# NIRVANALAN/CVPR23-E3DGE

Measured on AMD Instinct MI355X. Metric: rendered_rays_per_sec_64x64x24, higher is better.
Workload: dtype f32 (operands split f16 hi+lo, 3 f16 MFMA products, fp32 accumulate)

## Files before the change

cvpr23-e3dge_amd/csrc/siren16.h:

```cpp
#pragma once
#include "siren_common.h"

namespace e3dge {

typedef float f32x4v __attribute__((ext_vector_type(4)));

constexpr int k16Threads = 512;
constexpr int k16Tiles = 16;
constexpr int k16Steps = 8;
constexpr int k16ChunkFloats = 16 * kWidth;
constexpr int k16Chunks = kBigLayers * k16Tiles;
constexpr int k16NBuf = 4;
constexpr int k16Slots = 2;
constexpr int k16Ring = 2;

constexpr int k16LdsW = 0;
constexpr int k16LdsFilm = k16LdsW + k16NBuf * k16ChunkFloats;
constexpr int k16LdsHead = k16LdsFilm + 9 * 2 * kWidth;
constexpr int k16LdsW0 = k16LdsHead + kHeadFloats;
constexpr int k16LdsVrec = k16LdsW0 + 3 * kWidth;
constexpr int k16LdsFeat = k16LdsVrec + 2 * 4 * kWidth;
constexpr int k16LdsPart = k16LdsFeat + kRMax * kFPitch;
constexpr int k16LdsAlpha = ((k16LdsPart + 8 * k16Slots * kWidth + 3) / 4) * 4;
constexpr int k16LdsWgt = k16LdsAlpha + kTilePts;
constexpr int k16LdsZ = k16LdsWgt + kTilePts;
constexpr int k16LdsPts = k16LdsZ + kTilePts;
constexpr int k16LdsRgb = k16LdsPts + kTilePts * 3;
constexpr int k16LdsState = k16LdsRgb + kTilePts * 3;
constexpr int k16LdsWq = ((k16LdsState + kRMax * kStateStride + 3) / 4) * 4;
constexpr int k16LdsVd = k16LdsWq + 8 * k16Slots * 16;
constexpr int k16LdsFloats = k16LdsVd + 8 * 16 * 4;
constexpr int k16LdsBytes = k16LdsFloats * 4;
static_assert(k16LdsBytes <= 160 * 1024, "LDS budget");
static_assert((k16LdsFilm % 4) == 0 && (k16LdsHead % 4) == 0 && (k16LdsW0 % 4) == 0 && (k16LdsVrec % 4) == 0, "alignment");

__device__ __forceinline__ void save_st4(float* p, const f32x4v& v) {
    __builtin_nontemporal_store(v, reinterpret_cast<f32x4v*>(p));
}
__device__ __forceinline__ f32x4v mfma16x16(u32x4 a, u32x4 b, f32x4v c) {
    return __builtin_amdgcn_mfma_f32_16x16x32_f16(__builtin_bit_cast(half8, a), __builtin_bit_cast(half8, b), c, 0, 0, 0);
}
__device__ __forceinline__ f32x4v zero4() { return f32x4v{0.f, 0.f, 0.f, 0.f}; }
template <int HI> __device__ __forceinline__ float fma_mix_h(unsigned p, float w, float acc) {
    float r;
    if (HI) asm("v_fma_mix_f32 %0, %1, %2, %3 op_sel:[1,0,0] op_sel_hi:[1,0,0]" : "=v"(r) : "v"(p), "v"(w), "v"(acc));
    else asm("v_fma_mix_f32 %0, %1, %2, %3 op_sel:[0,0,0] op_sel_hi:[1,0,0]" : "=v"(r) : "v"(p), "v"(w), "v"(acc));
    return r;
}
__device__ __forceinline__ float act16_get(const u32x4 (&aH)[k16Steps], const u32x4 (&aL)[k16Steps], int t, int r) {
    const int g = t >> 1, w = 2 * (t & 1) + (r >> 1);
    return (r & 1) ? f16hi(aH[g][w]) + f16hi(aL[g][w]) : f16lo(aH[g][w]) + f16lo(aL[g][w]);
}
template <int CTRL> __device__ __forceinline__ float dpp16(float x) {
    return __builtin_bit_cast(float, __builtin_amdgcn_update_dpp(0, __builtin_bit_cast(int, x), CTRL, 0xf, 0xf, true));
}
__device__ __forceinline__ float row_sum16(float x) {
    x += dpp16<0x128>(x);
    x += dpp16<0x124>(x);
    x += dpp16<0x122>(x);
    x += dpp16<0x121>(x);
    return x;
}

__device__ __forceinline__ float sum_over_q(float x) {
    const unsigned u = __builtin_bit_cast(unsigned, x);
    const auto r = __builtin_amdgcn_permlane16_swap(u, u, false, false);
    const float y = __builtin_bit_cast(float, (unsigned)r[0]) + __builtin_bit_cast(float, (unsigned)r[1]);
    const unsigned v = __builtin_bit_cast(unsigned, y);
    const auto t = __builtin_amdgcn_permlane32_swap(v, v, false, false);
    return __builtin_bit_cast(float, (unsigned)t[0]) + __builtin_bit_cast(float, (unsigned)t[1]);
}

template <int CTRL, int ROW_MASK> __device__ __forceinline__ float dpp_or(float ident, float x) {
    return __builtin_bit_cast(float, __builtin_amdgcn_update_dpp(__builtin_bit_cast(int, ident), __builtin_bit_cast(int, x), CTRL, ROW_MASK, 0xf, false));
}
__device__ __forceinline__ float wave_incl_prod(float x) {
    x = __fmul_rn(x, dpp_or<0x111, 0xf>(1.0f, x));
    x = __fmul_rn(x, dpp_or<0x112, 0xf>(1.0f, x));
    x = __fmul_rn(x, dpp_or<0x114, 0xf>(1.0f, x));
    x = __fmul_rn(x, dpp_or<0x118, 0xf>(1.0f, x));
    x = __fmul_rn(x, dpp_or<0x142, 0xa>(1.0f, x));
    x = __fmul_rn(x, dpp_or<0x143, 0xc>(1.0f, x));
    return x;
}
__device__ __forceinline__ float wave_sum_last(float x) {
    x = __fadd_rn(x, dpp_or<0x111, 0xf>(0.0f, x));
    x = __fadd_rn(x, dpp_or<0x112, 0xf>(0.0f, x));
    x = __fadd_rn(x, dpp_or<0x114, 0xf>(0.0f, x));
    x = __fadd_rn(x, dpp_or<0x118, 0xf>(0.0f, x));
    x = __fadd_rn(x, dpp_or<0x142, 0xa>(0.0f, x));
    x = __fadd_rn(x, dpp_or<0x143, 0xc>(0.0f, x));
    return __builtin_bit_cast(float, __builtin_amdgcn_readlane(__builtin_bit_cast(int, x), 63));
}

struct ChunkPipe16 {
    const char* img;
    uint32_t voff, lds_base;
    int idx, buf, use_buf, count;
    float* wbuf;
    const float* wcur;
    const float* wnxt;
    __device__ __forceinline__ void init(float* wbuf_, const float* image, int wave, int lane, int count_ = k16Chunks) {
        const int wave_u = __builtin_amdgcn_readfirstlane(wave);
        wbuf = wbuf_;
        count = count_;
        img = reinterpret_cast<const char*>(image) + wave_u * 2048;
        voff = (uint32_t)lane * 16u;
        lds_base = (uint32_t)(size_t)(__attribute__((address_space(3))) float*)wbuf_ + (uint32_t)wave_u * 2048u;
        idx = 0; buf = 0; use_buf = 0;
        wcur = wbuf_; wnxt = wbuf_ + k16ChunkFloats;
    }
    __device__ __forceinline__ void issue_chunk() {
        const char* s = img + (size_t)idx * (k16ChunkFloats * 4);
        const uint32_t d = lds_base + (uint32_t)buf * (k16ChunkFloats * 4);
        glds16_saddr<0>(s, voff, d);
        glds16_saddr<1024>(s, voff, d);
        idx = (idx + 1 == count) ? 0 : idx + 1;
        buf = (buf + 1 == k16NBuf) ? 0 : buf + 1;
    }
    __device__ __forceinline__ void prime() {
        issue_chunk(); issue_chunk(); issue_chunk();
    }
#ifdef E3DGE_PHASE_TIMING
    unsigned long long t_vm = 0, t_bar = 0;
#endif
    template <bool STRICT> __device__ __forceinline__ void sync() {
#ifdef E3DGE_PHASE_TIMING
        const unsigned long long c0 = __builtin_readcyclecounter();
#endif
        if (STRICT) asm volatile("s_waitcnt vmcnt(0)" ::: "memory");
        else asm volatile("s_waitcnt vmcnt(2)" ::: "memory");
#ifdef E3DGE_PHASE_TIMING
        const unsigned long long c1 = __builtin_readcyclecounter();
#endif
        __syncthreads();
#ifdef E3DGE_PHASE_TIMING
        t_vm += c1 - c0; t_bar += __builtin_readcyclecounter() - c1;
#endif
    }
    __device__ __forceinline__ void advance() {
        use_buf = (use_buf + 1 == k16NBuf) ? 0 : use_buf + 1;
        wcur = wnxt;
        wnxt = wbuf + ((use_buf + 1 == k16NBuf) ? 0 : use_buf + 1) * k16ChunkFloats;
    }
};

#ifdef E3DGE_16_TRACE
__device__ unsigned long long g_trace16[2][24];
#define TRACE16_STAMP(i) do { if (trace) asm volatile("s_memtime %0" : "=s"(tstamp[i])); } while (0)
#else
#define TRACE16_STAMP(i) do { } while (0)
#endif

template <bool TRANSPOSED, int RING = k16Ring, class Epi, class Hook>
__device__ __forceinline__ void tile16(ChunkPipe16& pipe, int lane, const u32x4 (&aH)[k16Steps], const u32x4 (&aL)[k16Steps],
                                       f32x4v& acc, f32x4v& accb, u32x4 (&ringH)[RING], u32x4 (&ringL)[RING], Epi&& epi,
                                       Hook&& hook, int sbuf = -1, [[maybe_unused]] int trace = 0) {
#ifdef E3DGE_16_TRACE
    unsigned long long tstamp[24];
#endif
    const u32x4* __restrict__ wp = reinterpret_cast<const u32x4*>(sbuf >= 0 ? pipe.wbuf + sbuf * k16ChunkFloats : pipe.wcur) + lane;
    const u32x4* __restrict__ wn = reinterpret_cast<const u32x4*>(sbuf >= 0 ? pipe.wbuf + ((sbuf + 1) % k16NBuf) * k16ChunkFloats : pipe.wnxt) + lane;
#pragma unroll
    for (int g = 0; g < k16Steps; ++g) {
        const int ga = g + RING - 1;
        TRACE16_STAMP(3 * g);
        ringH[ga % RING] = (ga < k16Steps) ? wp[(ga * 2 + 0) * 64] : wn[((ga - k16Steps) * 2 + 0) * 64];
        ringL[ga % RING] = (ga < k16Steps) ? wp[(ga * 2 + 1) * 64] : wn[((ga - k16Steps) * 2 + 1) * 64];
        __builtin_amdgcn_sched_barrier(0);
        const u32x4 wh = ringH[g % RING], wl = ringL[g % RING];
        f32x4v& x0 = (g & 1) ? accb : acc;
        f32x4v& x1 = (g & 1) ? acc : accb;
        if (!TRANSPOSED) {
            x0 = mfma16x16(wh, aH[g], x0);
            x1 = mfma16x16(wl, aH[g], x1);
            x0 = mfma16x16(wh, aL[g], x0);
        } else {
            x0 = mfma16x16(aH[g], wh, x0);
            x1 = mfma16x16(aH[g], wl, x1);
            x0 = mfma16x16(aL[g], wh, x0);
        }
        TRACE16_STAMP(3 * g + 1);
        if (g == 1) hook();
        epi(g);
        TRACE16_STAMP(3 * g + 2);
    }
#ifdef E3DGE_16_TRACE
    if (trace) {
        asm volatile("s_waitcnt lgkmcnt(0)" ::: "memory");
        if ((threadIdx.x & 63) == 0)
            for (int i = 0; i < 24; ++i) g_trace16[trace - 1][i] = tstamp[i];
    }
#endif
}

#ifndef E3DGE_16_HELPERS_ONLY
#ifdef E3DGE_PHASE_TIMING
#define PHASE16(i) do { if (MODE == 0 && blockIdx.x == 0 && tid == 0 && sub < 3) tstamp[sub * 6 + (i)] = __builtin_readcyclecounter(); } while (0)
#else
#define PHASE16(i) do { } while (0)
#endif

constexpr int64_t k16SlabWords = 8 * 2 * 64;

template <int MODE, bool SAVE, int CACHE = 0>
__global__ void __launch_bounds__(k16Threads) siren16_kernel(const SirenK a) {
    static_assert(CACHE == 0 || (MODE == 0 && !SAVE), "the backbone hand-over exists for inference renders only");
    extern __shared__ __attribute__((aligned(16))) float smem[];
    float* const wbuf = smem + k16LdsW;
    float* const film_s = smem + k16LdsFilm;
    float* const head_s = smem + k16LdsHead;
    float* const w0_s = smem + k16LdsW0;
    float* const vrec_s = smem + k16LdsVrec;
    float* const feat_acc = smem + k16LdsFeat;
    float* const part = smem + k16LdsPart;
    float* const alpha_s = smem + k16LdsAlpha;
    float* const wgt_s = smem + k16LdsWgt;
    float* const z_s = smem + k16LdsZ;
    float* const pts_s = smem + k16LdsPts;
    float* const rgb_s = smem + k16LdsRgb;
    float* const state = smem + k16LdsState;

    const int tid_k = threadIdx.x;
#ifdef E3DGE_PHASE_TIMING
    const unsigned long long t_entry = __builtin_readcyclecounter();
    unsigned long long t_loop0 = 0, t_loop1 = 0;
#endif
    int b, npts, n_sub;
    int pix0 = 0, nrays = 0;
    long long pt0 = 0;
    const int S = (MODE == 0) ? a.S : 1;
    if (MODE == 0) {
        b = blockIdx.x / a.tiles_per_img;
        const int tile = blockIdx.x - b * a.tiles_per_img;
        const int HW = a.H * a.Wd;
        pix0 = tile * a.R;
        nrays = min(a.R, HW - pix0);
        npts = nrays * S;
    } else {
        b = blockIdx.x / a.wgs_per_img;
        const int wg = blockIdx.x - b * a.wgs_per_img;
        pt0 = (long long)wg * a.subtiles_per_wg * kTilePts;
        const long long rem = a.n_pts - pt0;
        npts = (int)(rem < (long long)a.subtiles_per_wg * kTilePts ? rem : (long long)a.subtiles_per_wg * kTilePts);
    }
    n_sub = (npts + kTilePts - 1) / kTilePts;

    const float* __restrict__ packed = a.packed;
    const float* __restrict__ film_g = a.film + (int64_t)b * 9 * 2 * kWidth;
    ChunkPipe16 pipe;
    if (CACHE == 2) pipe.init(wbuf, packed + kOffBig16b + (int64_t)(kBigLayers - 1) * k16Tiles * k16ChunkFloats, tid_k >> 6, tid_k & 63, k16Tiles);
    else pipe.init(wbuf, packed + kOffBig16b, tid_k >> 6, tid_k & 63);
    pipe.prime();
    constexpr int kFilmIt = (9 * kWidth + k16Threads - 1) / k16Threads;
    constexpr int kHeadIt = (kHeadFloats + k16Threads - 1) / k16Threads;
    constexpr int kColIt = (3 * kWidth + k16Threads - 1) / k16Threads;
    float ld_gm[kFilmIt], ld_bt[kFilmIt], ld_bias[kFilmIt], ld_head[kHeadIt], ld_w0[kColIt], ld_vt[kColIt];
#pragma unroll
    for (int j = 0; j < kFilmIt; ++j) {
        const int i = tid_k + j * k16Threads, l = i >> 8, n = i & 255;
        ld_gm[j] = ld_bt[j] = ld_bias[j] = 0.0f;
        if (i < 9 * kWidth) {
            ld_gm[j] = film_g[(l * 2 + 0) * kWidth + n];
            ld_bt[j] = film_g[(l * 2 + 1) * kWidth + n];
            ld_bias[j] = packed[kOffBias + l * kWidth + n];
        }
    }
#pragma unroll
    for (int j = 0; j < kHeadIt; ++j) {
        const int i = tid_k + j * k16Threads;
        ld_head[j] = (i < kHeadFloats) ? packed[kOffWSigma + i] : 0.0f;
    }
#pragma unroll
    for (int j = 0; j < kColIt; ++j) {
        const int i = tid_k + j * k16Threads, c = i >> 8, n = i & 255;
        const int src = ((n >> 5) * 2 + (c >> 1)) * 64 + (c & 1) * 32 + (n & 31);
        ld_w0[j] = ld_vt[j] = 0.0f;
        if (i < 3 * kWidth) { ld_w0[j] = packed[kOffFirst + src]; ld_vt[j] = packed[kOffVTail + src]; }
    }
#pragma unroll
    for (int j = 0; j < kFilmIt; ++j) {
        const int i = tid_k + j * k16Threads, l = i >> 8, n = i & 255;
        if (i < 9 * kWidth) {
            const float gm = ld_gm[j], bt = ld_bt[j];
            const float g_s = (l >= 1) ? gm * (1.0f / kW16Scale) : gm;
            const float b_s = __fadd_rn(__fmul_rn(gm, ld_bias[j]), bt);
            film_s[(l * 2 + 0) * kWidth + n] = g_s;
            film_s[(l * 2 + 1) * kWidth + n] = b_s;
            if (l == 8) { vrec_s[4 * n + 0] = g_s; vrec_s[4 * n + 1] = b_s; }
        }
    }
#pragma unroll
    for (int j = 0; j < kHeadIt; ++j) {
        const int i = tid_k + j * k16Threads;
        if (i < kHeadFloats) {
            head_s[i] = ld_head[j];
            const int c = (i >> 8) - 1, n = i & 255;
            if (c >= 0 && c < 3) vrec_s[(c == 2 ? 4 * kWidth : 0) + 4 * n + (c == 2 ? 0 : 2 + c)] = ld_head[j];
        }
    }
#pragma unroll
    for (int j = 0; j < kColIt; ++j) {
        const int i = tid_k + j * k16Threads, c = i >> 8, n = i & 255;
        if (i < 3 * kWidth) {
            w0_s[i] = ld_w0[j];
            vrec_s[4 * kWidth + 4 * n + 1 + c] = ld_vt[j] * kW16Scale;
        }
    }
    float cw[12] = {0}, focal = 1.f, nearv = 0.f, farv = 0.f;
    if (MODE == 0) {
#pragma unroll
        for (int i = 0; i < 12; ++i) cw[i] = a.c2w[b * 12 + i];
        focal = a.focal[b]; nearv = a.near[b]; farv = a.far[b];
        for (int i = tid_k; i < kRMax * kStateStride; i += k16Threads) state[i] = 0.0f;
        for (int i = tid_k; i < kRMax * kFPitch; i += k16Threads) feat_acc[i] = 0.0f;
    }
    const float* __restrict__ film = film_s;

    asm volatile("s_waitcnt vmcnt(0)" ::: "memory");
    __syncthreads();
    u32x4 ringH[k16Ring], ringL[k16Ring];
    {
        const int lane0 = tid_k & 63;
#pragma unroll
        for (int g = 0; g < k16Ring - 1; ++g) {
            ringH[g] = reinterpret_cast<const u32x4*>(pipe.wcur)[(g * 2 + 0) * 64 + lane0];
            ringL[g] = reinterpret_cast<const u32x4*>(pipe.wcur)[(g * 2 + 1) * 64 + lane0];
        }
    }

#ifdef E3DGE_16_TRACE
    auto trace_sel = [&](int L, int t) {
        const int w = __builtin_amdgcn_readfirstlane(tid_k >> 6);
        return (MODE == 0 && blockIdx.x == 7 && L == 3 && t == 6 && (w == 0 || w == 4)) ? 1 + (w >> 2) : 0;
    };
#else
    auto trace_sel = [](int, int) { return 0; };
#endif
    auto fwd_hook = [&](int younger) {
        if (SAVE) {
            switch (younger) {
                case 2: asm volatile("s_waitcnt vmcnt(2)" ::: "memory"); break;
                case 3: asm volatile("s_waitcnt vmcnt(3)" ::: "memory"); break;
                default: asm volatile("s_waitcnt vmcnt(4)" ::: "memory"); break;
            }
            asm volatile("s_waitcnt lgkmcnt(0)\n\ts_barrier" ::: "memory");
        } else {
            pipe.template sync<false>();
        }
        pipe.issue_chunk();
    };
    u32x4 inH[k16Steps], inL[k16Steps], outH[k16Steps], outL[k16Steps];
#ifdef E3DGE_PHASE_TIMING
    unsigned long long tstamp[18];
    for (int i = 0; i < 18; ++i) tstamp[i] = 0;
#endif

#ifdef E3DGE_PHASE_TIMING
    t_loop0 = __builtin_readcyclecounter();
#endif
    for (int sub = 0; sub < n_sub; ++sub) {
        int tid_o = tid_k;
        asm volatile("" : "+v"(tid_o));
        const int tid = tid_o, lane = tid & 63, wave = tid >> 6, q = lane >> 4, col = lane & 15;
        PHASE16(0);
        const int p_sub = 16 * wave + col;
        const int p = sub * kTilePts + p_sub;
        const bool valid = p < npts;
        const int pc = valid ? p : (npts - 1);
        float px = 0.f, py = 0.f, pz = 0.f, vx = 0.f, vy = 0.f, vz = 0.f, zval = 0.f, dist = 0.f;
        int ray_l = 0, s_idx = 0;
        int64_t gpt;
        if (MODE == 0) {
            ray_l = pc / S;
            s_idx = pc - ray_l * S;
            const int pix = pix0 + ray_l;
            const int iy = pix / a.Wd, ix = pix - iy * a.Wd;
            gpt = ((int64_t)b * a.H * a.Wd + pix) * S + s_idx;
            const float hres = (float)a.res * 0.5f;
            const float d0 = __fdiv_rn(((float)ix + 0.5f) - hres, focal);
            const float d1 = -__fdiv_rn(((float)iy + 0.5f) - hres, focal);
            const float d2 = -1.0f;
            float rd[3];
#pragma unroll
            for (int m = 0; m < 3; ++m)
                rd[m] = __fadd_rn(__fadd_rn(__fmul_rn(d0, cw[4 * m + 0]), __fmul_rn(d1, cw[4 * m + 1])), __fmul_rn(d2, cw[4 * m + 2]));
            const float dn = sqrtf(__fadd_rn(__fadd_rn(__fmul_rn(d0, d0), __fmul_rn(d1, d1)), __fmul_rn(d2, d2)));
            vx = __fdiv_rn(d0, dn); vy = __fdiv_rn(d1, dn); vz = __fdiv_rn(d2, dn);
            const float tv = a.t_vals[s_idx];
            zval = __fadd_rn(__fmul_rn(nearv, __fsub_rn(1.0f, tv)), __fmul_rn(farv, tv));
            px = __fadd_rn(cw[3], __fmul_rn(rd[0], zval));
            py = __fadd_rn(cw[7], __fmul_rn(rd[1], zval));
            pz = __fadd_rn(cw[11], __fmul_rn(rd[2], zval));
            const float rdn = sqrtf(__fadd_rn(__fadd_rn(__fmul_rn(rd[0], rd[0]), __fmul_rn(rd[1], rd[1])), __fmul_rn(rd[2], rd[2])));
            if (s_idx + 1 < S) {
                const float tn = a.t_vals[s_idx + 1];
                const float zn = __fadd_rn(__fmul_rn(nearv, __fsub_rn(1.0f, tn)), __fmul_rn(farv, tn));
                dist = __fmul_rn(__fsub_rn(zn, zval), rdn);
            } else {
                dist = __fmul_rn(1e10f, rdn);
            }
            if (valid && q == 0) {
                if (a.points) { float* o = a.points + gpt * 3; o[0] = px; o[1] = py; o[2] = pz; }
                if (a.dists) a.dists[gpt] = dist;
                if (s_idx == 0) {
                    const int64_t gr = (int64_t)b * a.H * a.Wd + pix;
                    if (a.rays_d) { float* o = a.rays_d + gr * 3; o[0] = rd[0]; o[1] = rd[1]; o[2] = rd[2]; }
                    if (a.viewdirs) { float* o = a.viewdirs + gr * 3; o[0] = vx; o[1] = vy; o[2] = vz; }
                }
            }
        } else {
            gpt = (int64_t)b * a.n_pts + pt0 + pc;
            const float* pp = a.pts + gpt * 3;
            px = pp[0]; py = pp[1]; pz = pp[2];
            if (a.vdirs) { const float* vv = a.vdirs + gpt * 3; vx = vv[0]; vy = vv[1]; vz = vv[2]; }
        }
        const int64_t gpt_block = (MODE == 0) ? ((int64_t)b * a.H * a.Wd + pix0) * S : (int64_t)b * a.n_pts + pt0;
        const bool sblk = SAVE && a.save_blocked != 0;
        const int64_t img_n = (MODE == 0) ? (int64_t)a.H * a.Wd * S : (int64_t)a.n_pts;
        const int64_t srow_block = (int64_t)b * saved_rows_per_image(sblk, img_n) + ((MODE == 0) ? (int64_t)pix0 * S : pt0);
        float* const sv = SAVE ? a.save_args + saved_row_floats(sblk, srow_block + pc, q, 9) : nullptr;
        const int sv_ls = sblk ? kSlabLayerF : kWidth, sv_ts = sblk ? kSlabTileF : 16;
        float* const vd_s = smem + k16LdsVd + wave * 64;
        if (q == 0) { vd_s[col * 4 + 0] = vx; vd_s[col * 4 + 1] = vy; vd_s[col * 4 + 2] = vz; }

        if (CACHE != 2) {
            const float xs = __fmul_rn(px, a.box_scale), ys = __fmul_rn(py, a.box_scale), zs = __fmul_rn(pz, a.box_scale);
#pragma unroll
            for (int t = 0; t < k16Tiles; ++t) {
                const int o = 16 * t + 4 * q;
                const f32x4v wx = *reinterpret_cast<const f32x4v*>(w0_s + o), wy = *reinterpret_cast<const f32x4v*>(w0_s + kWidth + o),
                             wz = *reinterpret_cast<const f32x4v*>(w0_s + 2 * kWidth + o);
                const f32x4v g4 = *reinterpret_cast<const f32x4v*>(film + o), b4 = *reinterpret_cast<const f32x4v*>(film + kWidth + o);
                f32x4v arg, v;
#pragma unroll
                for (int r = 0; r < 4; ++r) {
                    const float lin = fmaf(wz[r], zs, fmaf(wy[r], ys, wx[r] * xs));
                    arg[r] = fmaf(g4[r], lin, b4[r]);
                    v[r] = sin_f32(arg[r]);
                }
                if (SAVE) save_st4(sv + t * sv_ts, arg);
                SPLIT2_TO(v[0], v[1], inH[t >> 1][2 * (t & 1)], inL[t >> 1][2 * (t & 1)]);
                SPLIT2_TO(v[2], v[3], inH[t >> 1][2 * (t & 1) + 1], inL[t >> 1][2 * (t & 1) + 1]);
            }
        }

        PHASE16(1);
#pragma unroll 1
        for (int L = 1; L < ((CACHE == 2) ? 0 : E3DGE_SIREN_DEPTH); ++L) {
            const float* __restrict__ film_l = film + L * 2 * kWidth;
            f32x4v prev = zero4();
            auto finish = [&](int tp, const f32x4v& pv) {
                const int o = 16 * tp + 4 * q;
                const f32x4v g4 = *reinterpret_cast<const f32x4v*>(film_l + o), b4 = *reinterpret_cast<const f32x4v*>(film_l + kWidth + o);
                f32x4v arg, v;
#pragma unroll
                for (int r = 0; r < 4; ++r) { arg[r] = fmaf(g4[r], pv[r], b4[r]); v[r] = sin_f32(arg[r]); }
                if (SAVE) save_st4(sv + L * sv_ls + tp * sv_ts, arg);
                SPLIT2_TO(v[0], v[1], outH[tp >> 1][2 * (tp & 1)], outL[tp >> 1][2 * (tp & 1)]);
                SPLIT2_TO(v[2], v[3], outH[tp >> 1][2 * (tp & 1) + 1], outL[tp >> 1][2 * (tp & 1) + 1]);
            };
#pragma unroll
            for (int t = 0; t < k16Tiles; ++t) {
                f32x4v acc = zero4(), accb = zero4();
                if (t == 0) {
                    tile16<false>(pipe, lane, inH, inL, acc, accb, ringH, ringL, [](int) {}, [&]() { fwd_hook(2); }, t % k16NBuf);
                } else {
                    const int o = 16 * (t - 1) + 4 * q;
                    f32x4v g4 = zero4(), b4 = zero4(), arg4 = zero4(), kf4 = zero4(), x4 = zero4();
                    tile16<false>(pipe, lane, inH, inL, acc, accb, ringH, ringL, [&](int g) {
                        if (g == 0) {
                            g4 = *reinterpret_cast<const f32x4v*>(film_l + o);
                            b4 = *reinterpret_cast<const f32x4v*>(film_l + kWidth + o);
                        } else if (g == 1) {
#pragma unroll
                            for (int r = 0; r < 4; ++r) arg4[r] = fmaf(g4[r], prev[r], b4[r]);
#ifndef E3DGE_POLY_SINE
#pragma unroll
                            for (int r = 0; r < 4; ++r) kf4[r] = rintf(arg4[r] * 0.15915494f);
                        } else if (g == 2) {
#pragma unroll
                            for (int r = 0; r < 4; ++r) kf4[r] = fmaf(arg4[r], 6.4206382e-09f, fmaf(arg4[r], 0.15915494f, -kf4[r]));
#endif
                        } else if (g == 3) {
#pragma unroll
#ifndef E3DGE_POLY_SINE
                            for (int r = 0; r < 4; ++r) x4[r] = __builtin_amdgcn_sinf(kf4[r]);
#else
                            for (int r = 0; r < 4; ++r) x4[r] = sin_poly_f32(arg4[r]);
#endif
                            if (SAVE) save_st4(sv + L * sv_ls + (t - 1) * sv_ts, arg4);
                        } else if (g == 4) {
                            SPLIT2_TO(x4[0], x4[1], outH[(t - 1) >> 1][2 * ((t - 1) & 1)], outL[(t - 1) >> 1][2 * ((t - 1) & 1)]);
                            SPLIT2_TO(x4[2], x4[3], outH[(t - 1) >> 1][2 * ((t - 1) & 1) + 1], outL[(t - 1) >> 1][2 * ((t - 1) & 1) + 1]);
                        }
                    }, [&]() { fwd_hook(t < 2 ? 2 : (t == 2 ? 3 : 4)); }, t % k16NBuf, trace_sel(L, t));
                }
                pipe.advance();
                prev = acc + accb;
            }
            finish(k16Tiles - 1, prev);
#pragma unroll
            for (int g = 0; g < k16Steps; ++g) { inH[g] = outH[g]; inL[g] = outL[g]; }
        }

        if (CACHE != 0) {
            const int64_t rec = (((int64_t)blockIdx.x * a.bb_subs + sub) * 8 + wave) * k16SlabWords + lane;
            if (CACHE == 1) {
                u32x4* __restrict__ dst = reinterpret_cast<u32x4*>(a.bb_out) + rec;
#pragma unroll
                for (int g = 0; g < k16Steps; ++g) { dst[(g * 2 + 0) * 64] = inH[g]; dst[(g * 2 + 1) * 64] = inL[g]; }
            } else {
                const u32x4* __restrict__ src = reinterpret_cast<const u32x4*>(a.bb_in) + rec;
#pragma unroll
                for (int g = 0; g < k16Steps; ++g) { inH[g] = src[(g * 2 + 0) * 64]; inL[g] = src[(g * 2 + 1) * 64]; }
            }
        }

        PHASE16(2);
        float sdf = 0.0f;
        if (CACHE == 2) {
            if (q == 0) wgt_s[p_sub] = valid ? a.weights_in[gpt] : 0.0f;
        } else {
            float acc = 0.0f;
#pragma unroll
            for (int t = 0; t < k16Tiles; ++t) {
                const f32x4v w4 = *reinterpret_cast<const f32x4v*>(head_s + 16 * t + 4 * q);
                const int g = t >> 1, w0i = 2 * (t & 1);
                acc = fma_mix_h<0>(inH[g][w0i], w4[0], acc); acc = fma_mix_h<0>(inL[g][w0i], w4[0], acc);
                acc = fma_mix_h<1>(inH[g][w0i], w4[1], acc); acc = fma_mix_h<1>(inL[g][w0i], w4[1], acc);
                acc = fma_mix_h<0>(inH[g][w0i + 1], w4[2], acc); acc = fma_mix_h<0>(inL[g][w0i + 1], w4[2], acc);
                acc = fma_mix_h<1>(inH[g][w0i + 1], w4[3], acc); acc = fma_mix_h<1>(inL[g][w0i + 1], w4[3], acc);
            }
            sdf = sum_over_q(acc) + head_s[4 * kWidth];
        }

        if (MODE == 0 && CACHE != 2) {
            const float sg = __fdiv_rn(sigmoid_f32(__fdiv_rn(-sdf, a.sigmoid_beta)), a.sigmoid_beta);
            const float alpha = __fsub_rn(1.0f, expf(-__fmul_rn(sg, dist)));
            if (q == 0) {
                alpha_s[p_sub] = valid ? alpha : 0.0f;
                z_s[p_sub] = zval;
                pts_s[p_sub * 3 + 0] = px; pts_s[p_sub * 3 + 1] = py; pts_s[p_sub * 3 + 2] = pz;
                if (valid && a.sdf) a.sdf[gpt] = sdf;
            }
            __syncthreads();
            const int sub_lo = sub * kTilePts;
            const int sub_hi = min(sub_lo + kTilePts, npts);
            const int r_first = sub_lo / S, r_last = (sub_hi - 1) / S;
            for (int i = __builtin_amdgcn_readfirstlane(wave); i <= r_last - r_first; i += 8) {
                const int rl = r_first + i;
                const int s_lo = max(0, sub_lo - rl * S), s_hi = min(S, sub_hi - rl * S);
                float* st = state + rl * kStateStride;
                float T_in = (s_lo == 0) ? 1.0f : st[0];
                float wsum = (s_lo == 0) ? 0.0f : st[1];
                float dep = 0.0f, x0 = 0.0f, x1 = 0.0f, x2 = 0.0f;
                for (int c0 = s_lo; c0 < s_hi; c0 += 64) {
                    const int s = c0 + lane;
                    const bool act = s < s_hi;
                    const int ps = rl * S + min(s, s_hi - 1) - sub_lo;
                    const float al = act ? alpha_s[ps] : 0.0f;
                    const float zz = z_s[ps], p0 = pts_s[ps * 3 + 0], p1 = pts_s[ps * 3 + 1], p2 = pts_s[ps * 3 + 2];
                    const float incl = wave_incl_prod(act ? __fadd_rn(__fsub_rn(1.0f, al), 1e-10f) : 1.0f);
                    const float T = __fmul_rn(T_in, dpp_or<0x138, 0xf>(1.0f, incl));
                    float w = __fmul_rn(al, T);
                    const bool last = a.force_bg && act && s == S - 1;
                    const float wfront = wave_sum_last(last ? 0.0f : w);
                    if (last) w = __fsub_rn(1.0f, __fadd_rn(wsum, wfront));
                    wsum = __fadd_rn(wsum, wfront);
                    if (act) wgt_s[ps] = w;
                    dep = __fadd_rn(dep, wave_sum_last(__fmul_rn(w, zz)));
                    x0 = __fadd_rn(x0, wave_sum_last(__fmul_rn(w, p0)));
                    x1 = __fadd_rn(x1, wave_sum_last(__fmul_rn(w, p1)));
                    x2 = __fadd_rn(x2, wave_sum_last(__fmul_rn(w, p2)));
                    T_in = __fmul_rn(T_in, __builtin_bit_cast(float, __builtin_amdgcn_readlane(__builtin_bit_cast(int, incl), 63)));
                }
                if (lane == 0) {
                    st[0] = T_in; st[1] = wsum;
                    st[2] = __fadd_rn(st[2], dep); st[3] = __fadd_rn(st[3], x0); st[4] = __fadd_rn(st[4], x1); st[5] = __fadd_rn(st[5], x2);
                }
            }
            __syncthreads();
            if (valid && q == 0 && a.weights) a.weights[gpt] = wgt_s[p_sub];
        }

        if (MODE == 0 && a.tex_alpha) {
            const float* __restrict__ ta = a.tex_alpha + gpt * kWidth;
            const float* __restrict__ tb = a.tex_beta + gpt * kWidth;
#pragma unroll
            for (int t = 0; t < k16Tiles; ++t) {
                const f32x4v a4 = *reinterpret_cast<const f32x4v*>(ta + 16 * t + 4 * q);
                const f32x4v b4 = *reinterpret_cast<const f32x4v*>(tb + 16 * t + 4 * q);
                float y[4];
#pragma unroll
                for (int r = 0; r < 4; ++r) y[r] = __fadd_rn(__fmul_rn(__fadd_rn(a4[r], 1.0f), act16_get(inH, inL, t, r)), b4[r]);
                SPLIT2_TO(y[0], y[1], inH[t >> 1][2 * (t & 1)], inL[t >> 1][2 * (t & 1)]);
                SPLIT2_TO(y[2], y[3], inH[t >> 1][2 * (t & 1) + 1], inL[t >> 1][2 * (t & 1) + 1]);
            }
        }

        PHASE16(3);
        float* const wq_s = smem + k16LdsWq + wave * (k16Slots * 16);
        int slab_first_ray = 0, slab_nslots = 0;
        const int slab_p0 = sub * kTilePts + 16 * wave;
        if (MODE == 0) {
            const int slab_hi = min(slab_p0 + 16, npts);
            if (slab_hi > slab_p0) {
                slab_first_ray = slab_p0 / S;
                slab_nslots = (slab_hi - 1) / S - slab_first_ray + 1;
            }
            const int b1 = (slab_first_ray + 1) * S - slab_p0;
            if (lane < 16) {
                const float w = (slab_p0 + lane < npts) ? wgt_s[16 * wave + lane] : 0.0f;
                wq_s[lane] = (lane < b1) ? w : 0.0f;
                wq_s[16 + lane] = (lane >= b1) ? w : 0.0f;
            }
        }
        const f32x4v q0 = (MODE == 0) ? *reinterpret_cast<const f32x4v*>(wq_s + 4 * q) : zero4();
        const f32x4v q1 = (MODE == 0) ? *reinterpret_cast<const f32x4v*>(wq_s + 16 + 4 * q) : zero4();
        float dvx[4], dvy[4], dvz[4];
#pragma unroll
        for (int r = 0; r < 4; ++r) { dvx[r] = vd_s[(4 * q + r) * 4 + 0]; dvy[r] = vd_s[(4 * q + r) * 4 + 1]; dvz[r] = vd_s[(4 * q + r) * 4 + 2]; }
        float prgb[3][4];
#pragma unroll
        for (int c = 0; c < 3; ++c)
#pragma unroll
            for (int r = 0; r < 4; ++r) prgb[c][r] = 0.0f;
        {
            const f32x4v* __restrict__ vra = reinterpret_cast<const f32x4v*>(vrec_s) + col;
            const f32x4v* __restrict__ vrb = reinterpret_cast<const f32x4v*>(vrec_s + 4 * kWidth) + col;
            f32x4v ra = zero4(), rb = zero4(), pacc = zero4(), paccb = zero4(), pv = zero4(), varg = zero4(), kf = zero4(), hv = zero4();
            float fa0 = 0.f, fa1 = 0.f;
            auto epi = [&](int tp, int g) {
                const int e_n = 16 * tp + col;
                if (g == 0) {
                    const f32x4v s4 = pacc + paccb;
#pragma unroll
                    for (int r = 0; r < 4; ++r) pv[r] = fmaf(rb[3], dvz[r], fmaf(rb[2], dvy[r], fmaf(rb[1], dvx[r], s4[r])));
                } else if (g == 1) {
#pragma unroll
                    for (int r = 0; r < 4; ++r) varg[r] = fmaf(ra[0], pv[r], ra[1]);
#ifndef E3DGE_POLY_SINE
#pragma unroll
                    for (int r = 0; r < 4; ++r) kf[r] = rintf(varg[r] * 0.15915494f);
                } else if (g == 2) {
#pragma unroll
                    for (int r = 0; r < 4; ++r) kf[r] = fmaf(varg[r], 6.4206382e-09f, fmaf(varg[r], 0.15915494f, -kf[r]));
#pragma unroll
                    for (int r = 0; r < 4; ++r) hv[r] = __builtin_amdgcn_sinf(kf[r]);
#else
                } else if (g == 2) {
#pragma unroll
                    for (int r = 0; r < 4; ++r) hv[r] = sin_poly_f32(varg[r]);
#endif
                } else if (g == 3) {
#pragma unroll
                    for (int r = 0; r < 4; ++r) {
                        const int pr = slab_p0 + 4 * q + r;
                        if (SAVE && pr < npts) a.save_args[saved_elem_floats(sblk, srow_block + pr, 8, e_n, 9)] = varg[r];
                        if (MODE != 0 && a.raw && pr < npts) a.raw[((int64_t)b * a.n_pts + pt0 + pr) * 260 + 4 + e_n] = hv[r];
                    }
#pragma unroll
                    for (int r = 0; r < 4; ++r) {
                        prgb[0][r] = fmaf(ra[2], hv[r], prgb[0][r]);
                        prgb[1][r] = fmaf(ra[3], hv[r], prgb[1][r]);
                        prgb[2][r] = fmaf(rb[0], hv[r], prgb[2][r]);
                    }
                } else if (g == 4) {
                    if (MODE == 0) {
                        fa0 = fa1 = 0.f;
#pragma unroll
                        for (int r = 0; r < 4; ++r) { fa0 = fmaf(q0[r], hv[r], fa0); fa1 = fmaf(q1[r], hv[r], fa1); }
                    }
                } else if (g == 5) {
                    if (MODE == 0) {
                        fa0 = sum_over_q(fa0);
                        fa1 = sum_over_q(fa1);
                        if (q == 0) {
                            float* pp = part + (wave * k16Slots) * kWidth + e_n;
                            if (slab_nslots > 0) pp[0] = fa0;
                            if (slab_nslots > 1) pp[kWidth] = fa1;
                        }
                    }
                }
            };
            auto load_rec = [&](int t) { ra = vra[16 * t]; rb = vrb[16 * t]; };
            auto view_tile = [&](int t, int sbuf) {
                f32x4v acc = zero4(), accb = zero4();
                tile16<true>(pipe, lane, inH, inL, acc, accb, ringH, ringL, [&](int g) {
                    if (t > 0 && g <= 5) epi(t - 1, g);
                    if (g == 4) load_rec(t);
                }, [&]() { fwd_hook(2); }, sbuf);
                pipe.advance();
                pacc = acc; paccb = accb;
            };
            if constexpr (MODE == 0 && !SAVE) {
#pragma unroll
                for (int t = 0; t < k16Tiles; ++t) view_tile(t, t % k16NBuf);
            } else {
#pragma unroll 1
                for (int t = 0; t < k16Tiles; ++t) view_tile(t, -1);
            }
#pragma unroll
            for (int g = 0; g <= 5; ++g) epi(k16Tiles - 1, g);
        }

        PHASE16(4);
        float rgbv[3][4];
#pragma unroll
        for (int c = 0; c < 3; ++c)
#pragma unroll
            for (int r = 0; r < 4; ++r) rgbv[c][r] = row_sum16(prgb[c][r]) + head_s[4 * kWidth + 1 + c];
        if (MODE == 0) {
            if (col == 0) {
#pragma unroll
                for (int r = 0; r < 4; ++r) {
                    const int ps = 16 * wave + 4 * q + r;
                    rgb_s[ps * 3 + 0] = sigmoid_f32(rgbv[0][r]);
                    rgb_s[ps * 3 + 1] = sigmoid_f32(rgbv[1][r]);
                    rgb_s[ps * 3 + 2] = sigmoid_f32(rgbv[2][r]);
                }
            }
            __syncthreads();
            const int sub_lo = sub * kTilePts;
            const int sub_hi = min(sub_lo + kTilePts, npts);
            const int r_first = sub_lo / S, r_last = (sub_hi - 1) / S;
            for (int i = __builtin_amdgcn_readfirstlane(wave); i <= r_last - r_first; i += 8) {
                const int rl = r_first + i;
                const int s_lo = max(0, sub_lo - rl * S), s_hi = min(S, sub_hi - rl * S);
                float c0 = 0.0f, c1 = 0.0f, c2 = 0.0f;
                for (int b0 = s_lo; b0 < s_hi; b0 += 64) {
                    const int s = b0 + lane;
                    const int ps = rl * S + min(s, s_hi - 1) - sub_lo;
                    const float ww = (s < s_hi) ? wgt_s[ps] : 0.0f;
                    c0 = __fadd_rn(c0, wave_sum_last(__fmul_rn(ww, rgb_s[ps * 3 + 0])));
                    c1 = __fadd_rn(c1, wave_sum_last(__fmul_rn(ww, rgb_s[ps * 3 + 1])));
                    c2 = __fadd_rn(c2, wave_sum_last(__fmul_rn(ww, rgb_s[ps * 3 + 2])));
                }
                if (lane == 0) {
                    float* st = state + rl * kStateStride;
                    st[6] = __fadd_rn(st[6], c0); st[7] = __fadd_rn(st[7], c1); st[8] = __fadd_rn(st[8], c2);
                }
            }
            if (tid < kWidth) {
                const int n = tid;
                float pv[8 * k16Slots];
#pragma unroll
                for (int j = 0; j < 8 * k16Slots; ++j) pv[j] = part[j * kWidth + n];
                int cur = -1;
                float run = 0.0f;
#pragma unroll
                for (int wv = 0; wv < 8; ++wv) {
                    const int slab_lo = sub_lo + 16 * wv;
                    const int slab_hi2 = min(slab_lo + 16, npts);
                    if (slab_hi2 > slab_lo) {
                        const int fr = slab_lo / S;
                        const int ns = (slab_hi2 - 1) / S - fr + 1;
#pragma unroll
                        for (int sl = 0; sl < k16Slots; ++sl)
                            if (sl < ns) {
                                if (fr + sl != cur) {
                                    if (cur >= 0) feat_acc[cur * kFPitch + n] += run;
                                    cur = fr + sl;
                                    run = 0.0f;
                                }
                                run += pv[wv * k16Slots + sl];
                            }
                    }
                }
                if (cur >= 0) feat_acc[cur * kFPitch + n] += run;
            }
            __syncthreads();
        } else {
            if (a.raw && col == 0) {
#pragma unroll
                for (int r = 0; r < 4; ++r) {
                    const int pr = sub * kTilePts + 16 * wave + 4 * q + r;
                    if (pr < npts) {
                        float* o = a.raw + ((int64_t)b * a.n_pts + pt0 + pr) * 260;
                        o[0] = rgbv[0][r]; o[1] = rgbv[1][r]; o[2] = rgbv[2][r];
                    }
                }
            }
            if (valid && q == 0) {
                if (a.sdf) a.sdf[gpt] = sdf;
                if (a.raw) a.raw[gpt * 260 + 3] = sdf;
            }
        }
        PHASE16(5);
    }

#ifdef E3DGE_PHASE_TIMING
    t_loop1 = __builtin_readcyclecounter();
#endif
    asm volatile("s_waitcnt vmcnt(0)" ::: "memory");
    if (MODE == 0) {
        const int tid = tid_k;
        const int HW = a.H * a.Wd;
        if (a.features) {
            float* fo = a.features + (int64_t)b * kWidth * HW + pix0;
            for (int e = tid; e < nrays * kWidth; e += k16Threads) {
                const int n = e / nrays, rl = e - n * nrays;
                fo[(int64_t)n * HW + rl] = feat_acc[rl * kFPitch + n];
            }
        }
        for (int rl = tid; rl < nrays; rl += k16Threads) {
            const float* st = state + rl * kStateStride;
            const int pix = pix0 + rl;
            if (a.rgb) {
                float* o = a.rgb + (int64_t)b * 3 * HW + pix;
                o[0] = __fadd_rn(-1.0f, __fmul_rn(2.0f, st[6]));
                o[HW] = __fadd_rn(-1.0f, __fmul_rn(2.0f, st[7]));
                o[2 * HW] = __fadd_rn(-1.0f, __fmul_rn(2.0f, st[8]));
            }
            if (a.xyz) {
                float* o = a.xyz + (int64_t)b * 3 * HW + pix;
                o[0] = st[3]; o[HW] = st[4]; o[2 * HW] = st[5];
            }
            if (a.depth) a.depth[(int64_t)b * HW + pix] = st[2];
            if (a.mask) a.mask[(int64_t)b * HW + pix] = (st[2] < a.mask_thresh) ? 1.0f : 0.0f;
        }
#ifdef E3DGE_PHASE_TIMING
        __syncthreads();
        float* const td = a.dists ? a.dists : a.rgb;
        if (blockIdx.x == 0 && tid == 0 && td) {
            for (int i = 0; i < 18; ++i)
                td[i] = (i % 6 == 0) ? (float)(i / 6 ? tstamp[i] - tstamp[i - 1] : 0) : (float)(tstamp[i] - tstamp[i - 1]);
            td[18] = (float)pipe.t_vm; td[19] = (float)pipe.t_bar;
            td[20] = (float)(t_loop0 - t_entry);
            td[21] = (float)(t_loop1 - t_loop0);
            td[22] = (float)(__builtin_readcyclecounter() - t_loop1);
        }
#endif
    }
    asm volatile("s_waitcnt vmcnt(0)" ::: "memory");
}

__global__ void __launch_bounds__(64)
selftest_mfma16x16_kernel(float* __restrict__ cmat, const float* __restrict__ amat, const float* __restrict__ bmat, int k) {
    const int lane = threadIdx.x, q = lane >> 4, n = lane & 15;
    f32x4v acc = zero4();
    for (int kb = 0; kb < k; kb += 32) {
        u32x4 a4, b4, dummy;
#pragma unroll
        for (int w = 0; w < 4; ++w) {
            SPLIT2_TO(amat[n * k + kb + 8 * q + 2 * w], amat[n * k + kb + 8 * q + 2 * w + 1], a4[w], dummy[w]);
            SPLIT2_TO(bmat[n * k + kb + 8 * q + 2 * w], bmat[n * k + kb + 8 * q + 2 * w + 1], b4[w], dummy[w]);
        }
        acc = mfma16x16(a4, b4, acc);
    }
#pragma unroll
    for (int r = 0; r < 4; ++r) cmat[(4 * q + r) * 16 + n] = acc[r];
}

#endif

}
```

Baseline: 13.63 million.

## Overlap each layer's last-tile epilogue with the next layer's first MFMA tile

In the non-save render path, the last tile's FiLM and sine epilogue of each SIREN layer is deferred into the first tile of the next layer's MFMA pass, so the layer boundary no longer serialises on it. The input and output activation registers now ping-pong between layers instead of being copied back after each layer, and a reference alias picks the final buffer. The weight ring in LDS is also moved after the small tables so those tables stay within the ds_read immediate offset range. This adds control complexity and could raise register pressure.

```diff
diff --git a/cvpr23-e3dge_amd/csrc/siren16.h b/cvpr23-e3dge_amd/csrc/siren16.h
--- a/cvpr23-e3dge_amd/csrc/siren16.h
+++ b/cvpr23-e3dge_amd/csrc/siren16.h
@@ -14,12 +14,12 @@
 constexpr int k16Slots = 2;
 constexpr int k16Ring = 2;
 
-constexpr int k16LdsW = 0;
-constexpr int k16LdsFilm = k16LdsW + k16NBuf * k16ChunkFloats;
+constexpr int k16LdsFilm = 0;
 constexpr int k16LdsHead = k16LdsFilm + 9 * 2 * kWidth;
 constexpr int k16LdsW0 = k16LdsHead + kHeadFloats;
 constexpr int k16LdsVrec = k16LdsW0 + 3 * kWidth;
-constexpr int k16LdsFeat = k16LdsVrec + 2 * 4 * kWidth;
+constexpr int k16LdsW = k16LdsVrec + 2 * 4 * kWidth;
+constexpr int k16LdsFeat = k16LdsW + k16NBuf * k16ChunkFloats;
 constexpr int k16LdsPart = k16LdsFeat + kRMax * kFPitch;
 constexpr int k16LdsAlpha = ((k16LdsPart + 8 * k16Slots * kWidth + 3) / 4) * 4;
 constexpr int k16LdsWgt = k16LdsAlpha + kTilePts;
@@ -32,7 +32,8 @@
 constexpr int k16LdsFloats = k16LdsVd + 8 * 16 * 4;
 constexpr int k16LdsBytes = k16LdsFloats * 4;
 static_assert(k16LdsBytes <= 160 * 1024, "LDS budget");
-static_assert((k16LdsFilm % 4) == 0 && (k16LdsHead % 4) == 0 && (k16LdsW0 % 4) == 0 && (k16LdsVrec % 4) == 0, "alignment");
+static_assert((k16LdsFilm % 4) == 0 && (k16LdsHead % 4) == 0 && (k16LdsW0 % 4) == 0 && (k16LdsVrec % 4) == 0 && (k16LdsW % 4) == 0, "alignment");
+static_assert(k16LdsW * 4 <= 64 * 1024, "the tables stay inside the ds_read offset field");
 
 __device__ __forceinline__ void save_st4(float* p, const f32x4v& v) {
     __builtin_nontemporal_store(v, reinterpret_cast<f32x4v*>(p));
@@ -351,6 +352,10 @@
         pipe.issue_chunk();
     };
     u32x4 inH[k16Steps], inL[k16Steps], outH[k16Steps], outL[k16Steps];
+    constexpr bool kSeamless = MODE == 0 && !SAVE;
+    constexpr bool kFinalOut = kSeamless && ((E3DGE_SIREN_DEPTH - 1) & 1) != 0;
+    u32x4 (&hH)[k16Steps] = kFinalOut ? outH : inH;
+    u32x4 (&hL)[k16Steps] = kFinalOut ? outL : inL;
 #ifdef E3DGE_PHASE_TIMING
     unsigned long long tstamp[18];
     for (int i = 0; i < 18; ++i) tstamp[i] = 0;
@@ -424,6 +429,7 @@
         float* const vd_s = smem + k16LdsVd + wave * 64;
         if (q == 0) { vd_s[col * 4 + 0] = vx; vd_s[col * 4 + 1] = vy; vd_s[col * 4 + 2] = vz; }
 
+        f32x4v prev = zero4();
         if (CACHE != 2) {
             const float xs = __fmul_rn(px, a.box_scale), ys = __fmul_rn(py, a.box_scale), zs = __fmul_rn(pz, a.box_scale);
 #pragma unroll
@@ -431,47 +437,54 @@
                 const int o = 16 * t + 4 * q;
                 const f32x4v wx = *reinterpret_cast<const f32x4v*>(w0_s + o), wy = *reinterpret_cast<const f32x4v*>(w0_s + kWidth + o),
                              wz = *reinterpret_cast<const f32x4v*>(w0_s + 2 * kWidth + o);
-                const f32x4v g4 = *reinterpret_cast<const f32x4v*>(film + o), b4 = *reinterpret_cast<const f32x4v*>(film + kWidth + o);
-                f32x4v arg, v;
-#pragma unroll
-                for (int r = 0; r < 4; ++r) {
-                    const float lin = fmaf(wz[r], zs, fmaf(wy[r], ys, wx[r] * xs));
-                    arg[r] = fmaf(g4[r], lin, b4[r]);
-                    v[r] = sin_f32(arg[r]);
-                }
-                if (SAVE) save_st4(sv + t * sv_ts, arg);
-                SPLIT2_TO(v[0], v[1], inH[t >> 1][2 * (t & 1)], inL[t >> 1][2 * (t & 1)]);
-                SPLIT2_TO(v[2], v[3], inH[t >> 1][2 * (t & 1) + 1], inL[t >> 1][2 * (t & 1) + 1]);
+                f32x4v lin;
+#pragma unroll
+                for (int r = 0; r < 4; ++r) lin[r] = fmaf(wz[r], zs, fmaf(wy[r], ys, wx[r] * xs));
+                if (kSeamless && t == k16Tiles - 1) {
+                    prev = lin;
+                } else {
+                    const f32x4v g4 = *reinterpret_cast<const f32x4v*>(film + o), b4 = *reinterpret_cast<const f32x4v*>(film + kWidth + o);
+                    f32x4v arg, v;
+#pragma unroll
+                    for (int r = 0; r < 4; ++r) {
+                        arg[r] = fmaf(g4[r], lin[r], b4[r]);
+                        v[r] = sin_f32(arg[r]);
+                    }
+                    if (SAVE) save_st4(sv + t * sv_ts, arg);
+                    SPLIT2_TO(v[0], v[1], inH[t >> 1][2 * (t & 1)], inL[t >> 1][2 * (t & 1)]);
+                    SPLIT2_TO(v[2], v[3], inH[t >> 1][2 * (t & 1) + 1], inL[t >> 1][2 * (t & 1) + 1]);
+                }
             }
         }
 
         PHASE16(1);
-#pragma unroll 1
-        for (int L = 1; L < ((CACHE == 2) ? 0 : E3DGE_SIREN_DEPTH); ++L) {
-            const float* __restrict__ film_l = film + L * 2 * kWidth;
-            f32x4v prev = zero4();
-            auto finish = [&](int tp, const f32x4v& pv) {
-                const int o = 16 * tp + 4 * q;
-                const f32x4v g4 = *reinterpret_cast<const f32x4v*>(film_l + o), b4 = *reinterpret_cast<const f32x4v*>(film_l + kWidth + o);
-                f32x4v arg, v;
-#pragma unroll
-                for (int r = 0; r < 4; ++r) { arg[r] = fmaf(g4[r], pv[r], b4[r]); v[r] = sin_f32(arg[r]); }
-                if (SAVE) save_st4(sv + L * sv_ls + tp * sv_ts, arg);
-                SPLIT2_TO(v[0], v[1], outH[tp >> 1][2 * (tp & 1)], outL[tp >> 1][2 * (tp & 1)]);
-                SPLIT2_TO(v[2], v[3], outH[tp >> 1][2 * (tp & 1) + 1], outL[tp >> 1][2 * (tp & 1) + 1]);
-            };
+        auto finish = [&](const float* __restrict__ fl, int L, int tp, const f32x4v& pv, auto& dH, auto& dL) {
+            const int o = 16 * tp + 4 * q;
+            const f32x4v g4 = *reinterpret_cast<const f32x4v*>(fl + o), b4 = *reinterpret_cast<const f32x4v*>(fl + kWidth + o);
+            f32x4v arg, v;
+#pragma unroll
+            for (int r = 0; r < 4; ++r) { arg[r] = fmaf(g4[r], pv[r], b4[r]); v[r] = sin_f32(arg[r]); }
+            if (SAVE) save_st4(sv + L * sv_ls + tp * sv_ts, arg);
+            SPLIT2_TO(v[0], v[1], dH[tp >> 1][2 * (tp & 1)], dL[tp >> 1][2 * (tp & 1)]);
+            SPLIT2_TO(v[2], v[3], dH[tp >> 1][2 * (tp & 1) + 1], dL[tp >> 1][2 * (tp & 1) + 1]);
+        };
+        auto hidden_layer = [&](int L, auto& sH, auto& sL, auto& dH, auto& dL) {
+            const float* __restrict__ film_p = film + (L - 1) * 2 * kWidth;
 #pragma unroll
             for (int t = 0; t < k16Tiles; ++t) {
                 f32x4v acc = zero4(), accb = zero4();
-                if (t == 0) {
-                    tile16<false>(pipe, lane, inH, inL, acc, accb, ringH, ringL, [](int) {}, [&]() { fwd_hook(2); }, t % k16NBuf);
+                if (t == 0 && !kSeamless) {
+                    tile16<false>(pipe, lane, sH, sL, acc, accb, ringH, ringL, [](int) {}, [&]() { fwd_hook(2); }, t % k16NBuf);
                 } else {
-                    const int o = 16 * (t - 1) + 4 * q;
+                    const int tp = (t == 0) ? k16Tiles - 1 : t - 1;
+                    const int o = ((t == 0) ? 0 : 2 * kWidth) + 16 * tp + 4 * q;
+                    auto& eH = (t == 0) ? sH : dH;
+                    auto& eL = (t == 0) ? sL : dL;
                     f32x4v g4 = zero4(), b4 = zero4(), arg4 = zero4(), kf4 = zero4(), x4 = zero4();
-                    tile16<false>(pipe, lane, inH, inL, acc, accb, ringH, ringL, [&](int g) {
+                    tile16<false>(pipe, lane, sH, sL, acc, accb, ringH, ringL, [&](int g) {
                         if (g == 0) {
-                            g4 = *reinterpret_cast<const f32x4v*>(film_l + o);
-                            b4 = *reinterpret_cast<const f32x4v*>(film_l + kWidth + o);
+                            g4 = *reinterpret_cast<const f32x4v*>(film_p + o);
+                            b4 = *reinterpret_cast<const f32x4v*>(film_p + kWidth + o);
                         } else if (g == 1) {
 #pragma unroll
                             for (int r = 0; r < 4; ++r) arg4[r] = fmaf(g4[r], prev[r], b4[r]);
@@ -489,19 +502,35 @@
 #else
                             for (int r = 0; r < 4; ++r) x4[r] = sin_poly_f32(arg4[r]);
 #endif
-                            if (SAVE) save_st4(sv + L * sv_ls + (t - 1) * sv_ts, arg4);
+                            if (SAVE) save_st4(sv + L * sv_ls + tp * sv_ts, arg4);
                         } else if (g == 4) {
-                            SPLIT2_TO(x4[0], x4[1], outH[(t - 1) >> 1][2 * ((t - 1) & 1)], outL[(t - 1) >> 1][2 * ((t - 1) & 1)]);
-                            SPLIT2_TO(x4[2], x4[3], outH[(t - 1) >> 1][2 * ((t - 1) & 1) + 1], outL[(t - 1) >> 1][2 * ((t - 1) & 1) + 1]);
+                            SPLIT2_TO(x4[0], x4[1], eH[tp >> 1][2 * (tp & 1)], eL[tp >> 1][2 * (tp & 1)]);
+                            SPLIT2_TO(x4[2], x4[3], eH[tp >> 1][2 * (tp & 1) + 1], eL[tp >> 1][2 * (tp & 1) + 1]);
                         }
                     }, [&]() { fwd_hook(t < 2 ? 2 : (t == 2 ? 3 : 4)); }, t % k16NBuf, trace_sel(L, t));
                 }
                 pipe.advance();
                 prev = acc + accb;
             }
-            finish(k16Tiles - 1, prev);
-#pragma unroll
-            for (int g = 0; g < k16Steps; ++g) { inH[g] = outH[g]; inL[g] = outL[g]; }
+        };
+        if constexpr (kSeamless) {
+            if (CACHE != 2) {
+#pragma unroll 1
+                for (int L = 1; L < E3DGE_SIREN_DEPTH; L += 2) {
+                    hidden_layer(L, inH, inL, outH, outL);
+                    if (L + 1 >= E3DGE_SIREN_DEPTH) break;
+                    hidden_layer(L + 1, outH, outL, inH, inL);
+                }
+                finish(film + (E3DGE_SIREN_DEPTH - 1) * 2 * kWidth, E3DGE_SIREN_DEPTH - 1, k16Tiles - 1, prev, hH, hL);
+            }
+        } else {
+#pragma unroll 1
+            for (int L = 1; L < E3DGE_SIREN_DEPTH; ++L) {
+                hidden_layer(L, inH, inL, outH, outL);
+                finish(film + L * 2 * kWidth, L, k16Tiles - 1, prev, outH, outL);
+#pragma unroll
+                for (int g = 0; g < k16Steps; ++g) { inH[g] = outH[g]; inL[g] = outL[g]; }
+            }
         }
 
         if (CACHE != 0) {
@@ -509,11 +538,11 @@
             if (CACHE == 1) {
                 u32x4* __restrict__ dst = reinterpret_cast<u32x4*>(a.bb_out) + rec;
 #pragma unroll
-                for (int g = 0; g < k16Steps; ++g) { dst[(g * 2 + 0) * 64] = inH[g]; dst[(g * 2 + 1) * 64] = inL[g]; }
+                for (int g = 0; g < k16Steps; ++g) { dst[(g * 2 + 0) * 64] = hH[g]; dst[(g * 2 + 1) * 64] = hL[g]; }
             } else {
                 const u32x4* __restrict__ src = reinterpret_cast<const u32x4*>(a.bb_in) + rec;
 #pragma unroll
-                for (int g = 0; g < k16Steps; ++g) { inH[g] = src[(g * 2 + 0) * 64]; inL[g] = src[(g * 2 + 1) * 64]; }
+                for (int g = 0; g < k16Steps; ++g) { hH[g] = src[(g * 2 + 0) * 64]; hL[g] = src[(g * 2 + 1) * 64]; }
             }
         }
 
@@ -527,10 +556,10 @@
             for (int t = 0; t < k16Tiles; ++t) {
                 const f32x4v w4 = *reinterpret_cast<const f32x4v*>(head_s + 16 * t + 4 * q);
                 const int g = t >> 1, w0i = 2 * (t & 1);
-                acc = fma_mix_h<0>(inH[g][w0i], w4[0], acc); acc = fma_mix_h<0>(inL[g][w0i], w4[0], acc);
-                acc = fma_mix_h<1>(inH[g][w0i], w4[1], acc); acc = fma_mix_h<1>(inL[g][w0i], w4[1], acc);
-                acc = fma_mix_h<0>(inH[g][w0i + 1], w4[2], acc); acc = fma_mix_h<0>(inL[g][w0i + 1], w4[2], acc);
-                acc = fma_mix_h<1>(inH[g][w0i + 1], w4[3], acc); acc = fma_mix_h<1>(inL[g][w0i + 1], w4[3], acc);
+                acc = fma_mix_h<0>(hH[g][w0i], w4[0], acc); acc = fma_mix_h<0>(hL[g][w0i], w4[0], acc);
+                acc = fma_mix_h<1>(hH[g][w0i], w4[1], acc); acc = fma_mix_h<1>(hL[g][w0i], w4[1], acc);
+                acc = fma_mix_h<0>(hH[g][w0i + 1], w4[2], acc); acc = fma_mix_h<0>(hL[g][w0i + 1], w4[2], acc);
+                acc = fma_mix_h<1>(hH[g][w0i + 1], w4[3], acc); acc = fma_mix_h<1>(hL[g][w0i + 1], w4[3], acc);
             }
             sdf = sum_over_q(acc) + head_s[4 * kWidth];
         }
@@ -593,9 +622,9 @@
                 const f32x4v b4 = *reinterpret_cast<const f32x4v*>(tb + 16 * t + 4 * q);
                 float y[4];
 #pragma unroll
-                for (int r = 0; r < 4; ++r) y[r] = __fadd_rn(__fmul_rn(__fadd_rn(a4[r], 1.0f), act16_get(inH, inL, t, r)), b4[r]);
-                SPLIT2_TO(y[0], y[1], inH[t >> 1][2 * (t & 1)], inL[t >> 1][2 * (t & 1)]);
-                SPLIT2_TO(y[2], y[3], inH[t >> 1][2 * (t & 1) + 1], inL[t >> 1][2 * (t & 1) + 1]);
+                for (int r = 0; r < 4; ++r) y[r] = __fadd_rn(__fmul_rn(__fadd_rn(a4[r], 1.0f), act16_get(hH, hL, t, r)), b4[r]);
+                SPLIT2_TO(y[0], y[1], hH[t >> 1][2 * (t & 1)], hL[t >> 1][2 * (t & 1)]);
+                SPLIT2_TO(y[2], y[3], hH[t >> 1][2 * (t & 1) + 1], hL[t >> 1][2 * (t & 1) + 1]);
             }
         }
 
@@ -687,7 +716,7 @@
             auto load_rec = [&](int t) { ra = vra[16 * t]; rb = vrb[16 * t]; };
             auto view_tile = [&](int t, int sbuf) {
                 f32x4v acc = zero4(), accb = zero4();
-                tile16<true>(pipe, lane, inH, inL, acc, accb, ringH, ringL, [&](int g) {
+                tile16<true>(pipe, lane, hH, hL, acc, accb, ringH, ringL, [&](int g) {
                     if (t > 0 && g <= 5) epi(t - 1, g);
                     if (g == 4) load_rec(t);
                 }, [&]() { fwd_hook(2); }, sbuf);
```

After: 13.77 million, median of 6. +1.0%, better.
